# KyungMinJin/OTPose

Hardware: AMD Instinct MI355X
Metric: frames/sec at 384x288, 5-frame window, batch 16; heatmap max-abs delta vs ref (higher is better)
Workload: dtype f32 storage+accumulate / f16x3 split products; 1 GPU; BASELINE configs[1]: batch 16 x 5-frame x 384x288, HRNet-W48 + DCN warp + ConvVideoTransformer, fp32 forward (eval), seeded synthetic weights; clips_per_gpu=16, parallelism=dp1, outputs_finite=True

## Files before the change

include/otpose_hip.h:

```cpp
#ifndef OTPOSE_HIP_H
#define OTPOSE_HIP_H

#include <stddef.h>

#ifdef __cplusplus
extern "C" {
#endif

#define OTP_OK 0
#define OTP_ERR_BAD_ARG (-1)
#define OTP_ERR_UNSUPPORTED (-2)
#define OTP_ERR_LAUNCH (-3)
#define OTP_ERR_WORKSPACE (-4)

#define OTP_DTYPE_F32 0
#define OTP_DTYPE_F16 1
#define OTP_DTYPE_BF16 2
#define OTP_DTYPE_F64 3

#define OTP_ACT_NONE 0
#define OTP_ACT_RELU 1
#define OTP_ACT_GELU 2

int otp_version(void);
// ... 101 lines not shown
int otp_conv3x3_small_supported(const otp_conv_desc* desc);
size_t otp_conv3x3_small_weight_bytes(int Cout, int Cin);
int otp_conv3x3_small_pack(const void* weight, void* wpacked, int Cout, int Cin, void* stream);
int otp_conv3x3_small(const void* in, const void* in2, const void* wpacked, const void* scale, const void* shift, void* out,
                      const otp_conv_desc* desc, void* stream);

size_t otp_conv2d_x3_weight_bytes(int Cout, int Cin, int k, int stride);
int otp_conv2d_x3_pack_weight(const void* weight, const void* scale, void* wpacked, int Cout, int Cin, int k, int stride,
                              void* stream);
int otp_conv2d_x3_supported(const otp_conv_desc* desc);
int otp_conv2d_x3(const void* in, const void* wpacked, const void* shift, const void* res, void* out,
                  const otp_conv_desc* desc, void* stream);

#define OTP_S8_F32_C4 1
#define OTP_S8_F32_NCHW 2
size_t otp_s8_bytes(int N, int C, int H, int W);
int otp_s8_pack(const void* in_f32, void* out_s8, void* out_c4, int N, int C, int H, int W, int in_ctot, int in_coff, void* stream);
int otp_s8_upsample_add(const void* const* lows, const int* factors, int nlow, const void* res, void* out_nchw, void* out_s8,
                        void* out_c4, int N, int C, int Hh, int Wh, int relu, int res_ctot, int res_coff, int out_ctot,
                        int out_coff, void* stream);
int otp_s8_upsample_add_ex(const void* const* lows, const int* factors, int nlow, const void* res, int res_layout, void* out_nchw,
                           void* out_s8, void* out_c4, int N, int C, int Hh, int Wh, int relu, int res_ctot, int res_coff,
                           int out_ctot, int out_coff, void* stream);
int otp_s8_unpack(const void* in_s8, void* out_f32, int N, int C, int H, int W, void* stream);
int otp_c4_unpack(const void* in_c4, void* out_f32, int N, int C, int H, int W, void* stream);
int otp_conv3x3_s8_supported(const otp_conv_desc* desc);
size_t otp_conv3x3_s8_weight_bytes(int Cout, int Cin);
int otp_conv3x3_s8_pack_weight(const void* weight, const void* scale, void* wpacked, int Cout, int Cin, void* stream);
int otp_conv3x3_s8(const void* in_s8, const void* wpacked, const void* shift, const void* res_c4, void* out_f32,
                   int out_f32_layout, void* out_s8, const otp_conv_desc* desc, void* stream);
int otp_conv3x3_s2_s8_supported(const otp_conv_desc* desc, int nchw_out);
int otp_conv3x3_s2_s8(const void* in_s8, const void* wpacked, const void* shift, const void* res_nchw, void* out_nchw,
                      void* out_s8, const otp_conv_desc* desc, void* stream);

int otp_conv2d_pack_weight_dgrad(const void* weight, void* wpacked, int Cout, int Cin, int kh, int kw, void* stream);
int otp_dilate(const void* in, void* out, int planes, int Hi, int Wi, int s, int H, int W, void* stream);
size_t otp_conv2d_wgrad_workspace(int Cin, int Cout);
int otp_conv2d_wgrad(const void* x, const void* grad_out, void* grad_weight, int N, int Cin, int H, int W, int Cout,
                     int kh, int kw, int stride, int pad, int dil, int x_ctot, int x_coff, int dy_ctot, int dy_coff,
                     void* workspace, size_t workspace_bytes, void* stream);
size_t otp_bn_workspace(int N, int C, int HW);
int otp_bn_train_forward(const void* x, const void* gamma, const void* beta, const void* res, void* y, void* save_mean,
                         void* save_rstd, void* running_mean, void* running_var, void* workspace, size_t workspace_bytes,
                         int N, int C, int HW, float eps, float momentum, int relu, int x_ctot, int x_coff, int res_ctot,
                         int res_coff, int y_ctot, int y_coff, void* stream);
int otp_bn_train_backward(const void* grad_y, const void* x, const void* y_relu, const void* save_mean,
                          const void* save_rstd, const void* gamma, void* grad_x, void* grad_res, void* grad_gamma,
                          void* grad_beta, void* workspace, size_t workspace_bytes, int N, int C, int HW, int dy_ctot,
                          int dy_coff, int x_ctot, int x_coff, int y_ctot, int y_coff, void* stream);
int otp_channel_sum(const void* a, void* out, void* workspace, size_t workspace_bytes, int N, int C, int HW, int a_ctot,
                    int a_coff, void* stream);

int otp_dcn_fused_supported(int Cin, int J, int H, int W, int ND);
size_t otp_dcn_fused_weight_bytes(int ND, int J);
int otp_dcn_fused_pack(const void* const* w_off, const void* const* w_mask, const void* const* w_dcn, const void* const* bias,
                       void* packed, int ND, int J, void* stream);
size_t otp_dcn_fused_workspace(int B, int H, int W);
int otp_dcn_fused_forward(const void* trans, const void* x, const void* packed, void* out, void* workspace,
                          size_t workspace_bytes, int B, int Cin, int J, int H, int W, const int* dilations, int ND, float alpha,
                          void* stream);

int otp_glue_total(const void* rough, void* total, void* squeezed, void* inter, void* flow_in, const void* pe,
                   int B, int J, int HW, void* stream);
int otp_glue_stack(const void* rough, const void* margin, const void* squeezed, const void* inter,
                   const void* ctx, const void* pe1, const void* pe2, void* x1, void* x2, void* prev_b,
                   int B, int J, int HW, void* stream);
// ... 249 lines not shown
```

otpose_amd/csrc/convs2.hip:

```cpp
#include "x3.h"
#include <cstdlib>

namespace {

constexpr int MAXJ = 4;

struct S2Plan {
    int N, C, H, W, HW, Ho, Wo, HWo, Cout, total;
    int out_ctot, out_coff, res_ctot, res_coff, act;
    float pre, post;
    int NTW, nN, nTiles, nChunks, tpx, NPT;
    int VR, W1, NIW, NV, pl;
    uint32_t mHWo, mWo, mW1, mVR;
    unsigned* rflag;
};

template <int NTW, bool NCHW, int NPT>
__global__ __launch_bounds__(256, 2) void convs2_kernel(const unsigned char* __restrict__ xs, const otp_u32x4* __restrict__ wpk,
                                                         const float* __restrict__ shift, const float* res, float* outf,
                                                         otp_u32x4* outs, const S2Plan P) {
    constexpr int BM = 64 * NPT;
    constexpr int WCH = otp_s8_wch(NTW);
    constexpr int WBYTES = WCH * 1024;
    constexpr int NBLK = OTP_S8_KS * NPT;
    constexpr int NM = 3 * NTW;
    extern __shared__ __attribute__((aligned(16))) unsigned char smem[];
    const int PL = P.pl;
    unsigned char* win = smem;
    unsigned char* wl = smem + 4 * PL;
    const int tid = threadIdx.x, lane = tid & 63;
    const int wave = __builtin_amdgcn_readfirstlane(tid >> 6);
    const int i16 = lane & 15, kl = lane >> 4;
    const bool upper = kl >= 2;

    const int xcd = (int)blockIdx.x & 7, jb = (int)blockIdx.x >> 3;
    const int tl_ = jb / P.nN, cb = jb - tl_ * P.nN;
    const int tile = xcd * P.tpx + tl_;
    if (tile >= P.nTiles) return;
    const int P0 = tile * BM;
    const int n0 = P0 / P.HWo, p0 = P0 - n0 * P.HWo;
    const int y0 = (int)otp_magic_div((uint32_t)p0, P.mWo);
    const int Vf = n0 * P.VR + 2 * y0;
    const int imgB = P.C * P.HW * 4;
    const int co_blk = cb * NTW * 16;

    int voff[MAXJ];
    bool vlive[MAXJ];
#pragma unroll
    for (int j = 0; j < MAXJ; ++j) {
        const int v = 64 * (wave + 4 * j) + lane;
        vlive[j] = v < P.NV;
        const int r = (int)otp_magic_div((uint32_t)v, P.mW1), i = v - r * P.W1;
        const int V = Vf + r;
// ... 98 lines not shown
            const bool nb = blk + 2 < NBLK;
            const bool na = (NPT >= 2 ? p == NPT - 2 : true) && s + 1 < OTP_S8_KS;
            if (nb) load_b((blk + 2) % 3, blk + 2);
            if (na) load_a(sa ^ 1, s + 1);
#pragma unroll
            for (int t = 0; t < NTW; ++t) {
                acc[t][p] = OTP_X3_MFMA(al[sa][t], bh[cur], acc[t][p], 0, 0, 0);
                acc[t][p] = OTP_X3_MFMA(ah[sa][t], bl[cur], acc[t][p], 0, 0, 0);
                acc[t][p] = OTP_X3_MFMA(ah[sa][t], bh[cur], acc[t][p], 0, 0, 0);
            }
            if (!nb && !na) otp_s8_block_sched<NM, 0>();
            else if (nb && na) otp_s8_block_sched<NM, 2 + 2 * NTW>();
            else if (na) otp_s8_block_sched<NM, 2 * NTW>();
            else otp_s8_block_sched<NM, 2>();
            __builtin_amdgcn_sched_barrier(0);
        }
    };

    for (int c = 0; c < P.nChunks; ++c) {
        asm volatile("s_waitcnt vmcnt(0)" ::: "memory");
        __syncthreads();
        mfma_phase();
        if (c + 1 < P.nChunks) {
            __syncthreads();
            stage(c + 1);
        }
    }

    if (P.post != 1.f) {
#pragma unroll
        for (int t = 0; t < NTW; ++t)
#pragma unroll
            for (int p = 0; p < NPT; ++p) acc[t][p] = acc[t][p] * P.post;
    }
    if (!NCHW) {
        {
            bool bad = false;
#pragma unroll
            for (int t = 0; t < NTW; ++t)
#pragma unroll
                for (int p = 0; p < NPT; ++p)
#pragma unroll
                    for (int r = 0; r < 4; ++r) bad |= otp_out_of_range(acc[t][p][r]);
            otp_range_report(P.rflag, bad, OTP_RANGE_CONVS2);
        }
        if (P.act == OTP_ACT_RELU) {
#pragma unroll
            for (int t = 0; t < NTW; ++t)
#pragma unroll
                for (int p = 0; p < NPT; ++p)
#pragma unroll
                    for (int r = 0; r < 4; ++r) acc[t][p][r] = otp_relu(acc[t][p][r]);
        }
        otp_u32x4 rec[(NTW + 1) / 2][NPT][2];
#pragma unroll
        for (int t = 0; t < NTW; t += 2) {
            const bool paired = otp_tile_paired(co_blk, t, NTW, P.Cout);
            const int t1 = t + 1 < NTW ? t + 1 : t;
#pragma unroll
            for (int p = 0; p < NPT; ++p) {
                const float f[8] = {acc[t][p][0], acc[t][p][1], acc[t][p][2], acc[t][p][3],
                                    paired ? acc[t1][p][0] : 0.f, paired ? acc[t1][p][1] : 0.f,
                                    paired ? acc[t1][p][2] : 0.f, paired ? acc[t1][p][3] : 0.f};
                otp_x3_split8(f, rec[t >> 1][p][0], rec[t >> 1][p][1]);
            }
        }
// ... 108 lines not shown
        const int NV = window_records(P, bm);
        size_t lds = (size_t)4 * NV * 16 + otp_s8_wch(P.NTW) * 1024;
        if (nchw && lds < (size_t)P.NTW * 16 * (bm + 4) * 4) lds = (size_t)P.NTW * 16 * (bm + 4) * 4;
        if (NV <= 64 * 4 * MAXJ && lds <= 80 * 1024) {
            P.NV = NV;
            found = true;
            if ((long)P.nTiles * P.nN >= 2 * 256 || npt == 1) break;
        }
    }
    if (!found) return false;
    {
        const int bm = 64 * P.NPT;
        P.nTiles = (P.total + bm - 1) / bm;
        P.NV = window_records(P, bm);
        if (P.NV > 64 * 4 * MAXJ) return false;
    }
    P.tpx = (P.nTiles + 7) / 8;
    P.pl = P.NV * 16;
    P.NIW = (P.NV + 63) / 64;
    P.mHWo = otp_magic(P.HWo); P.mWo = otp_magic(Wo); P.mW1 = otp_magic(P.W1); P.mVR = otp_magic(P.VR);
    if ((long)(P.HWo + 256) * P.HWo >= (1l << 32) || (long)P.HWo * Wo >= (1l << 32)) return false;
    if ((long)(d.N + 2) * P.VR * P.VR >= (1l << 32) || (long)(64 * 4 * MAXJ) * P.W1 >= (1l << 32)) return false;
    {
        const long span = (long)(64 * P.NPT) / P.HWo + 2;
        if (span * d.Cin * P.HW * 4 >= (1l << 31)) return false;
    }
    if ((size_t)d.N * d.out_ctot * P.HWo * 4 >= (1ull << 31) || (size_t)d.N * (d.res_ctot > 0 ? d.res_ctot : 1) * P.HWo * 4 >= (1ull << 31))
        return false;
    if ((size_t)P.nN * P.nChunks * otp_s8_wch(P.NTW) * 1024 >= (1ull << 31)) return false;
    if (P.HWo < 16) return false;
    return true;
}

template <int NTW, bool NCHW, int NPT>
int convs2_launch(const void* xs, const void* wpk, const float* shift, const float* res, float* outf, void* outs, const S2Plan& P,
                  hipStream_t st) {
    auto kern = convs2_kernel<NTW, NCHW, NPT>;
    size_t need = (size_t)4 * P.pl + otp_s8_wch(NTW) * 1024;
    if (NCHW && need < (size_t)NTW * 16 * (64 * NPT + 4) * 4) need = (size_t)NTW * 16 * (64 * NPT + 4) * 4;
    OTP_ALLOW_BIG_LDS(kern, need);
    hipLaunchKernelGGL(kern, dim3(8 * P.tpx * P.nN), dim3(256), need, st, static_cast<const unsigned char*>(xs),
                       static_cast<const otp_u32x4*>(wpk), shift, res, outf, static_cast<otp_u32x4*>(outs), P);
    return otp_launch_status();
}

}

extern "C" int otp_conv3x3_s2_s8_supported(const otp_conv_desc* desc, int nchw_out) {
    if (!desc) return 0;
    S2Plan P{};
    return convs2_plan(*desc, P, nchw_out != 0) ? 1 : 0;
}

extern "C" int otp_conv3x3_s2_s8(const void* in_s8, const void* wpacked, const void* shift, const void* res_nchw, void* out_nchw,
                                 void* out_s8, const otp_conv_desc* desc, void* stream) {
    if (!in_s8 || !wpacked || !desc || (!out_nchw) == (!out_s8)) return OTP_ERR_BAD_ARG;
    if (res_nchw && !out_nchw) return OTP_ERR_BAD_ARG;
    const otp_conv_desc& d = *desc;
    if (d.N <= 0 || d.Cin <= 0 || d.Cout <= 0 || d.H <= 0 || d.W <= 0) return OTP_ERR_BAD_ARG;
    if (out_nchw && d.out_ctot < d.out_coff + d.Cout) return OTP_ERR_BAD_ARG;
    if (res_nchw && d.res_ctot < d.res_coff + d.Cout) return OTP_ERR_BAD_ARG;
    if ((reinterpret_cast<uintptr_t>(in_s8) | reinterpret_cast<uintptr_t>(wpacked) | reinterpret_cast<uintptr_t>(out_nchw) |
         reinterpret_cast<uintptr_t>(out_s8) | reinterpret_cast<uintptr_t>(res_nchw) | reinterpret_cast<uintptr_t>(shift)) & 15)
        return OTP_ERR_UNSUPPORTED;
    S2Plan P{};
    const bool nchw = out_nchw != nullptr;
    if (!convs2_plan(d, P, nchw)) return OTP_ERR_UNSUPPORTED;
    P.rflag = otp_range_word();
    auto st = static_cast<hipStream_t>(stream);
    auto fs = static_cast<const float*>(shift);
    auto fr = static_cast<const float*>(res_nchw);
    auto fo = static_cast<float*>(out_nchw);
#define OTP_C2_GO(NTW_, NCHW_, NPT_) return convs2_launch<NTW_, NCHW_, NPT_>(in_s8, wpacked, fs, fr, fo, out_s8, P, st)
#define OTP_C2_NPT(NPT_)                                                     \
    if (P.NPT == NPT_) {                                                     \
        if (P.NTW == 2) { if (nchw) OTP_C2_GO(2, true, NPT_); OTP_C2_GO(2, false, NPT_); } \
        if (nchw) OTP_C2_GO(3, true, NPT_);                                  \
        OTP_C2_GO(3, false, NPT_);                                           \
    }
    OTP_C2_NPT(4)
    OTP_C2_NPT(2)
    OTP_C2_NPT(1)
#undef OTP_C2_NPT
#undef OTP_C2_GO
    return OTP_ERR_UNSUPPORTED;
}
```

otpose_amd/engine.py:

```python
from __future__ import annotations

import ctypes
import dataclasses
import os
import sys
import warnings
from typing import Callable, List, Optional, Tuple

import torch

from . import hip, ops
from .ops import ACT_GELU, ACT_NONE, ACT_RELU, View

def _pair(v):
    return (int(v), int(v)) if isinstance(v, int) else (int(v[0]), int(v[1]))


def plain_conv(cv, k, stride=1, pad="same", dil=1, groups=1, bias=False, cin=None, cout=None) -> bool:
    if pad == "same":
        pad = (dil or 1) * (k // 2)
    return (cv.kernel_size == (k, k) and (stride is None or cv.stride == (stride, stride))
            and (pad is None or tuple(cv.padding) == (pad, pad)) and (dil is None or tuple(cv.dilation) == (dil, dil))
            and (groups is None or cv.groups == groups) and (bias is None or (cv.bias is not None) == bias)
            and (cin is None or cv.in_channels == cin) and (cout is None or cv.out_channels == cout))
# ... 61 lines not shown
    def __init__(self, s8=None, c4=None, nchw_needed=False):
        self.s8, self.c4, self.nchw_needed = s8, c4, nchw_needed


class InferenceEngine:
    h16 = False

    def __init__(self, model, batch: int, device, use_graph: bool | None = None, stream_set: int = 0, inp=None, margin=None):
        routes = Routes.from_env()
        self._init(device, routes, routes.use_graph if use_graph is None else use_graph, stream_set)
        self.B = batch
        self.model = model
        cfg = model.cfg
        self.J = model.num_joints
        self.F = getattr(model, "window_frames", 5)
        self.W_img, self.H_img = cfg.MODEL.IMAGE_SIZE
        self.h, self.w = model.pe_h, model.pe_w
        self._given = (inp, margin)
        self.param_version = self._param_version()
        with torch.no_grad():
            self._build()

    def _init(self, device, routes: Routes, use_graph: bool, stream_set: int = 0):
        device = torch.device(device)
        if device.type != "cuda" or not torch.cuda.is_available():
            raise RuntimeError("otpose_amd.OTPose runs on an MI355X through libotpose_hip.so; "
                               f"got device '{device}' (there is no CPU or PyTorch-op fallback)")
        self.lib, self.dev, self.routes = hip.lib(), device, routes
        self.model, self.B, self.inp, self.margin = None, 0, None, None
        self.ops: List[Callable] = []
        self._pair_s8 = {}
        self.l1_pairs = 0
        self._aux = {}
        self._keep = []
        self._bufs = []
        self._stream = None
        self.use_graph, self.graph = use_graph, None
        self._exact = False
        self._sid = 0
        self._side = hip.side_streams(device, 3, 4 * stream_set) if routes.multi_stream else []

    @classmethod
    def bare(cls, device, multi_stream=False):
        self = cls.__new__(cls)
        self._init(device, dataclasses.replace(Routes.from_env(), multi_stream=bool(multi_stream)), use_graph=False)
        return self

    use_x3 = property(lambda self: self.routes.use_x3)
    use_dcn_fused = property(lambda self: self.routes.use_dcn_fused)
    multi_stream = property(lambda self: self.routes.multi_stream)
    f32_tail = property(lambda self: self.routes.f32_tail)
    range_check = property(lambda self: self.routes.range_check)
    half_products = property(lambda self: self.h16 and self.routes.use_x3 and self.routes.h16_tail)

    @property
    def s8_here(self) -> bool:
        return self.routes.use_s8 and not self._exact

    @property
    def s2_here(self) -> bool:
        return self.routes.use_s8 and not self._exact and self.routes.s8_stride2

    def matches(self, x) -> bool:
        return (x.shape[0] == self.B and x.device == self.dev and tuple(x.shape[2:]) == (self.H_img, self.W_img)
                and self._param_version() == self.param_version)

# ... 32 lines not shown
        return cin >= 32 and cin % 8 == 0 and cout16 >= 48 and ((cout16 + 47) // 48) * 48 <= 1.15 * cout16

    def _emit(self, fn):
        self.ops.append((fn, self._sid))

    def fork(self, sids):
        if not self.multi_stream:
            return
        sids = [s for s in sids if 0 < s <= len(self._side)]

        def run():
            main = torch.cuda.current_stream(self.dev)
            for s_ in sids:
                self._side[s_ - 1].wait_stream(main)
        self.ops.append((run, -1))

    def join(self, sids):
        if not self.multi_stream:
            return
        sids = [s for s in sids if 0 < s <= len(self._side)]

        def run():
            main = torch.cuda.current_stream(self.dev)
            for s_ in sids:
                main.wait_stream(self._side[s_ - 1])
        self.ops.append((run, -1))

    def on_stream(self, sid):
        self._sid = sid if (self.multi_stream and 0 <= sid <= len(self._side)) else 0

    def call(self, fn, name, *args):
        def run():
            hip.check(fn(*args, self._stream), name)
        self._emit(run)

    def call_lazy_nchw(self, aux: Aux, fn, name, args_of, unpack=None):
        full, lean = args_of(True), args_of(False)
        if unpack is None:
            def run():
                hip.check(fn(*(full if aux.nchw_needed else lean), self._stream), name)
        else:
            s8_unpack = self.lib.otp_s8_unpack

            def run():
                hip.check(fn(*lean, self._stream), name)
                if aux.nchw_needed:
                    hip.check(s8_unpack(*unpack, self._stream), "otp_s8_unpack")
        self._emit(run)

    def _bn_fold(self, bn, bias=None):
        g, b = self.dev_param(bn.weight), self.dev_param(bn.bias)
        mu, var = self.dev_param(bn.running_mean), self.dev_param(bn.running_var)
        sc = (g / torch.sqrt(var + bn.eps)).contiguous()
        sh = b - mu * sc
        if bias is not None:
            sh = sh + self.dev_param(bias) * sc
        sh = sh.contiguous()
        self._keep += [sc, sh]
        return sc, sh

    def conv(self, inp: View, weight, out: View, stride=1, pad=0, dil=1, bn=None, bias=None, act=ACT_NONE,
             res: View = None, in2: View = None, res_up=1, frame_split=0, cin=None, scale=None, shift=None):
        for v_ in (inp, in2, res):
            self._needs_nchw(v_)
        r = self.routes
        w = self.dev_param(weight)
        if w.dim() == 3:
            w = w.unsqueeze(-1)
        cout, cin_w, kh, kw = w.shape
        if bn is not None:
# ... 75 lines not shown

    def fuse_s8(self, lows, factors, res: View, tgt: View):
        n_, c_, hh, wh = tgt.t.shape
        if not self.s8_here or tgt.coff != 0 or tgt.C != c_ or c_ % 16 or wh % 4 or (hh * wh) % 4:
            return False
        if not ops.s8_conv_supported(ops.s8_conv_desc(n_, c_, c_, hh, wh, ACT_RELU)):
            return False
        r = self.routes
        raux = self._aux.get(id(res.t)) if (r.lazy_nchw and res.coff == 0 and res.C == c_ and res.ctot == c_) else None
        res_img = raux.s8 if raux is not None else None
        if res_img is None:
            self._needs_nchw(res)
        s8 = self.new(n_ * c_ * hh * wh)
        c4 = None if r.s8_residual else self.new(n_ * c_ * hh * wh)
        aux = self._aux[id(tgt.t)] = Aux(s8, c4)
        lp = (ctypes.c_void_p * len(lows))(*[hip.ptr(v.t) for v in lows])
        fp = (ctypes.c_int * len(lows))(*factors)
        self._keep += [lp, fp]
        self.call_lazy_nchw(aux, self.lib.otp_s8_upsample_add_ex, "otp_s8_upsample_add", lambda nchw: (
            lp, fp, len(lows), hip.ptr(res_img if res_img is not None else res.t), int(res_img is not None),
            hip.ptr(tgt.t) if nchw else None, hip.ptr(s8), hip.ptr(c4), n_, c_, hh, wh, 1, res.ctot, res.coff, tgt.ctot, tgt.coff))
        return True

    def s8_image(self, v: View, want_c4=False):
        n, c, h, w = v.t.shape
        if not self.routes.use_s8 or v.coff != 0 or v.C != c or c % 16 or (h * w) % 4:
            return None
        aux = self._aux.get(id(v.t))
        if aux is not None and aux.s8 is not None and (not want_c4 or aux.c4 is not None):
            return aux
        self._needs_nchw(v)
        s8 = aux.s8 if aux is not None and aux.s8 is not None else self.new(n * c * h * w)
        c4 = self.new(n * c * h * w) if want_c4 else None
        self.call(self.lib.otp_s8_pack, "otp_s8_pack", hip.ptr(v.t), hip.ptr(s8), hip.ptr(c4), n, c, h, w, v.ctot, v.coff)
        if aux is None:
            aux = self._aux[id(v.t)] = Aux(nchw_needed=True)
        aux.s8 = s8
        if c4 is not None:
            aux.c4 = c4
        return aux

    def s2_chain_s8(self, layers, x: View, act_last, res: View = None, out: View = None):
        if not self.s2_here:
            return None
        n, c, h, w = x.t.shape
        if x.coff != 0 or x.C != c:
            return None
        hh, ww, cin = h, w, c
        descs = []
        for li, (cv, bn, relu) in enumerate(layers):
            last = li == len(layers) - 1
            if not plain_conv(cv, 3, stride=2, cin=cin) or hh % 2 or ww % 2:
                return None
            co = cv.out_channels
            if last:
                if out is None:
                    out = View(self.new(n, co, hh // 2, ww // 2))
                d = ops.s8_s2_conv_desc(n, cin, co, hh, ww, act_last, out, res)
            else:
                d = ops.s8_s2_conv_desc(n, cin, co, hh, ww, ACT_RELU if relu else ACT_NONE)
            if not ops.s8_s2_conv_supported(d, last):
                return None
            descs.append(d)
            hh, ww, cin = hh // 2, ww // 2, co
        aux = self.s8_image(x)
        if aux is None:
            return None
        self._needs_nchw(res)
        cur = aux.s8
        hh, ww = h, w
        for (cv, bn, relu), d in zip(layers, descs):
            wp, sh = self._pack_s8(cv, bn, d)
            if d is descs[-1]:
                args = ops.conv3x3_s2_s8_args(cur, wp, sh, d, res, out)
            else:
                nxt = self.new(n * cv.out_channels * (hh // 2) * (ww // 2))
                args = ops.conv3x3_s2_s8_args(cur, wp, sh, d, out_s8=nxt)
                cur = nxt
            self.call(self.lib.otp_conv3x3_s2_s8, "otp_conv3x3_s2_s8", *args)
            hh, ww = hh // 2, ww // 2
        return out

    def _pack_s8(self, conv, bn, desc):
        sc, sh = self._bn_fold(bn)
        w = self.dev_param(conv.weight)
        e = ops.x3_weight_exponent(w, sc)
        desc.out_scale = 2.0 ** -e
        wp = ops.pack_s8_weight(w, sc, e)
        self._keep += [wp, desc]
        return wp, sh

    def conv_s8(self, x8, conv, bn, d, **outputs):
        wp, sh = self._pack_s8(conv, bn, d)
        self.call(self.lib.otp_conv3x3_s8, "otp_conv3x3_s8", *ops.conv3x3_s8_args(x8, wp, sh, d, **outputs))

    def conv_s8_lazy(self, x8, conv, bn, d, out: View, o8, res=None):
        wp, sh = self._pack_s8(conv, bn, d)
        aux = Aux(o8, nchw_needed=o8 is None or not self.routes.lazy_nchw)
        if o8 is not None:
            self._aux[id(out.t)] = aux
        self.call_lazy_nchw(aux, self.lib.otp_conv3x3_s8, "otp_conv3x3_s8", lambda nchw: ops.conv3x3_s8_args(
            x8, wp, sh, d, res, out.t if nchw else None, ops.S8_F32_NCHW, o8))

    def branch_s8(self, blocks, x: View, want_s8=False):
        n, c, h, w = x.t.shape
        if not self.s8_here or x.coff != 0 or x.C != c:
            return None
        for blk in blocks:
            convs = (getattr(blk, "conv1", None), getattr(blk, "conv2", None))
            if (getattr(blk, "downsample", None) is not None or hasattr(blk, "conv3")
                    or any(cv is None or not plain_conv(cv, 3, cin=c, cout=c) for cv in convs)):
                return None
        if not ops.s8_conv_supported(ops.s8_conv_desc(n, c, c, h, w, ACT_RELU)):
# ... 124 lines not shown
            sc, sh = self._bn_fold(blk.bn3)
            out = self.pointx_pair(y, c3.weight, sc, sh, res, nxt)
            if out is not None:
                return out
        return self.conv_bn(y, blk.conv3, blk.bn3, ACT_RELU, res=res)

    def hr_module(self, mod, xs: List[View], fork_in=True, join_out=True) -> List[View]:
        n = mod.num_branches
        xs = list(xs)
        r = self.routes
        if fork_in:
            self.fork(range(1, n))
        for i in range(n):
            self.on_stream(i)
            y = self.branch_s8(list(mod.branches[i]), xs[i], want_s8=i < len(mod.fuse_layers) - 1 and self.s2_here)
            if y is not None:
                xs[i] = y
                continue
            for blk in mod.branches[i]:
                xs[i] = self.basic_block(blk, xs[i])
        self.on_stream(0)
        self.join(range(1, n))
        if n == 1:
            return xs
        outs = []
        if self.s2_here:
            for j in range(min(n, len(mod.fuse_layers) - 1)):
                self.s8_image(xs[j])
        self.fork(range(1, len(mod.fuse_layers)))
        for i in range(len(mod.fuse_layers)):
            self.on_stream(i)
            terms = [j for j in range(n) if j != i]
            y = None
            ups = [j for j in terms if j > i]
            hi_w = xs[i].t.shape[3]
            if r.fuse_upsample and len(ups) >= 2 and hi_w % 4 == 0:
                terms = [j for j in terms if j < i]
            else:
                ups = []
            for idx, j in enumerate(terms):
                last = idx == len(terms) - 1 and not ups
                act = ACT_RELU if last else ACT_NONE
                res = xs[i] if y is None else y
                fl = mod.fuse_layers[i][j]
                tgt = y if y is not None else View(self.new(*xs[i].t.shape))
                if j > i:
                    f = 2 ** (j - i)
                    if f >= 2 and ((xs[j].t.shape[3] * f) % 4 == 0 or r.up_any_width):
                        low = self.conv_bn(xs[j], fl[0], fl[1], ACT_NONE)
                        if act == ACT_RELU and low.coff == 0 and low.C == low.ctot and self.fuse_s8([low], [f], res, tgt):
                            y = tgt
                            continue
                        self._needs_nchw(res)
                        self.call(self.lib.otp_upsample_add, "otp_upsample_add", *ops.upsample_add_args(low, res, tgt, f, act == ACT_RELU))
                        y = tgt
                    else:
                        y = self.conv_bn(xs[j], fl[0], fl[1], act, res=res, out=tgt, res_up=f)
                else:
                    chain = [(fl[k][0], fl[k][1], k < len(fl) - 1) for k in range(len(fl))]
                    if self.s2_chain_s8(chain, xs[j], act, res=res, out=tgt) is not None:
                        y = tgt
                        continue
                    t = xs[j]
                    for k in range(len(fl) - 1):
                        t = self.conv_bn(t, fl[k][0], fl[k][1], ACT_RELU)
                    y = self.conv_bn(t, fl[-1][0], fl[-1][1], act, res=res, out=tgt)
            if ups:
                res = xs[i] if y is None else y
                tgt = y if y is not None else View(self.new(*xs[i].t.shape))
                lows = [self.conv_bn(xs[j], mod.fuse_layers[i][j][0], mod.fuse_layers[i][j][1], ACT_NONE) for j in ups]
                factors = [2 ** (j - i) for j in ups]
                if self.fuse_s8(lows, factors, res, tgt):
                    outs.append(tgt)
                    continue
                self._needs_nchw(res)
                args, arrays = ops.upsample_add_multi_args(lows, factors, res, tgt, relu=True)
                self._keep += arrays
                self.call(self.lib.otp_upsample_add_multi, "otp_upsample_add_multi", *args)
                y = tgt
            outs.append(y)
        self.on_stream(0)
        if join_out:
            self.join(range(1, len(mod.fuse_layers)))
        return outs

    def hr_stages(self, net, x, width_change, new_branch, module, before_fork=None):
        ys = [x]
        for s in (2, 3, 4):
            trans = getattr(net, f"transition{s - 1}")
            live = [i for i, tr in enumerate(trans) if tr is not None]
            if before_fork is not None:
                before_fork(s, ys)
            self.fork(range(1, len(live)))
            xs = []
            for i, tr in enumerate(trans):
                if tr is None:
                    xs.append(ys[i])
                    continue
                self.on_stream(live.index(i))
                if isinstance(tr[0], torch.nn.Conv2d):
                    xs.append(width_change(s, ys[i], tr))
                else:
                    xs.append(new_branch(s, ys[-1], tr))
            self.on_stream(0)
            self.join(range(1, len(live)))
            ys = xs
            mods = list(getattr(net, f"stage{s}"))
            cont = False
            for mi, mod in enumerate(mods):
                fork_in, nxt = not cont, (mods[mi + 1] if mi + 1 < len(mods) else None)
                cont = (self.routes.chain_modules and nxt is not None and len(mod.fuse_layers) == nxt.num_branches
                        and mod.num_branches > 1)
                ys = module(s, mi, len(mods), mod, ys, fork_in, not cont)
        return ys

    def hrnet(self, net, x_in: View) -> View:
        c1 = net.conv1
# ... 393 lines not shown
```

otpose_amd/hip.py:

```python
from __future__ import annotations

import ctypes
import os
import threading
from ctypes import c_float, c_int, c_size_t, c_void_p

_HERE = os.path.dirname(os.path.abspath(__file__))
LIB_PATH = os.environ.get("OTPOSE_HIP_LIB") or os.path.join(_HERE, "csrc", "libotpose_hip.so")
_lib = None
_tls = threading.local()

OTP_OK = 0
_ERRORS = {
    -1: "OTP_ERR_BAD_ARG (null pointer or non-positive dimension)",
    -2: "OTP_ERR_UNSUPPORTED (shape / dtype / stride combination not implemented)",
    -3: "OTP_ERR_LAUNCH (HIP launch error)",
    -4: "OTP_ERR_WORKSPACE (workspace too small)",
}


class ConvDesc(ctypes.Structure):
    _fields_ = [(n, c_int) for n in (
        "N", "Cin", "H", "W", "Cout", "kh", "kw", "stride", "pad", "dil",
        "in_ctot", "in_coff", "in2_ctot", "in2_coff", "out_ctot", "out_coff",
# ... 47 lines not shown
    "otp_mdcn_backward": (c_int, [c_void_p] * 10 + [c_void_p, c_size_t] + [c_int] * 12 + [c_int, c_void_p]),
    "otp_deform_psroi_pool_forward": (c_int, [c_void_p] * 5 + [c_int] * 7 + [c_float] + [c_int] * 5 + [c_float, c_int, c_void_p]),
    "otp_deform_psroi_pool_backward_workspace": (c_size_t, [c_int] * 13),
    "otp_deform_psroi_pool_backward": (c_int, [c_void_p] * 7 + [c_int] * 7 + [c_float] + [c_int] * 5 + [c_float]
                                       + [c_void_p, c_size_t, c_int, c_void_p]),
    "otp_conv2d_pack_weight": (c_int, [c_void_p, c_void_p, c_int, c_int, c_int, c_int, c_void_p]),
    "otp_conv2d": (c_int, [c_void_p] * 7 + [ctypes.POINTER(ConvDesc), c_void_p]),
    "otp_conv2d_wino_weight_bytes": (c_size_t, [c_int, c_int]),
    "otp_conv2d_wino_pack_weight": (c_int, [c_void_p, c_void_p, c_int, c_int, c_void_p]),
    "otp_conv2d_wino_supported": (c_int, [ctypes.POINTER(ConvDesc)]),
    "otp_conv2d_wino_last_plan": (c_int, [ctypes.POINTER(c_int)]),
    "otp_conv2d_wino": (c_int, [c_void_p] * 6 + [ctypes.POINTER(ConvDesc), c_void_p]),
    "otp_conv3x3_small_supported": (c_int, [ctypes.POINTER(ConvDesc)]),
    "otp_conv3x3_small_weight_bytes": (c_size_t, [c_int, c_int]),
    "otp_conv3x3_small_pack": (c_int, [c_void_p, c_void_p, c_int, c_int, c_void_p]),
    "otp_conv3x3_small": (c_int, [c_void_p] * 6 + [ctypes.POINTER(ConvDesc), c_void_p]),
    "otp_conv2d_x3_weight_bytes": (c_size_t, [c_int, c_int, c_int, c_int]),
    "otp_conv2d_x3_pack_weight": (c_int, [c_void_p, c_void_p, c_void_p, c_int, c_int, c_int, c_int, c_void_p]),
    "otp_conv2d_x3_supported": (c_int, [ctypes.POINTER(ConvDesc)]),
    "otp_conv2d_x3": (c_int, [c_void_p] * 5 + [ctypes.POINTER(ConvDesc), c_void_p]),
    "otp_s8_bytes": (c_size_t, [c_int] * 4),
    "otp_s8_pack": (c_int, [c_void_p] * 3 + [c_int] * 6 + [c_void_p]),
    "otp_s8_upsample_add": (c_int, [ctypes.POINTER(c_void_p), ctypes.POINTER(c_int), c_int] + [c_void_p] * 4 + [c_int] * 9 + [c_void_p]),
    "otp_s8_upsample_add_ex": (c_int, [ctypes.POINTER(c_void_p), ctypes.POINTER(c_int), c_int, c_void_p, c_int] + [c_void_p] * 3
                               + [c_int] * 9 + [c_void_p]),
    "otp_s8_unpack": (c_int, [c_void_p, c_void_p] + [c_int] * 4 + [c_void_p]),
    "otp_c4_unpack": (c_int, [c_void_p, c_void_p] + [c_int] * 4 + [c_void_p]),
    "otp_conv3x3_s8_supported": (c_int, [ctypes.POINTER(ConvDesc)]),
    "otp_conv3x3_s8_weight_bytes": (c_size_t, [c_int, c_int]),
    "otp_conv3x3_s8_pack_weight": (c_int, [c_void_p] * 3 + [c_int, c_int, c_void_p]),
    "otp_conv3x3_s8": (c_int, [c_void_p] * 5 + [c_int, c_void_p, ctypes.POINTER(ConvDesc), c_void_p]),
    "otp_conv3x3_s2_s8_supported": (c_int, [ctypes.POINTER(ConvDesc), c_int]),
    "otp_conv3x3_s2_s8": (c_int, [c_void_p] * 6 + [ctypes.POINTER(ConvDesc), c_void_p]),
    "otp_conv2d_set_tile": (c_int, [c_int] * 4),
    "otp_conv2d_last_plan": (c_int, [ctypes.POINTER(c_int)]),
    "otp_conv2d_plan": (c_int, [ctypes.POINTER(ConvDesc), ctypes.POINTER(c_int)]),
    "otp_conv2d_pack_weight_dgrad": (c_int, [c_void_p, c_void_p, c_int, c_int, c_int, c_int, c_void_p]),
    "otp_dilate": (c_int, [c_void_p, c_void_p] + [c_int] * 6 + [c_void_p]),
    "otp_grad_sumsq_scratch": (c_size_t, []),
    "otp_grad_sumsq": (c_int, [c_void_p, c_size_t, c_void_p, c_void_p]),
    "otp_adamw_step": (c_int, [c_void_p] * 4 + [c_size_t] + [c_float] * 5 + [c_int, c_void_p, c_float, c_void_p]),
    "otp_pck_accuracy": (c_int, [c_void_p] * 4 + [c_int] * 4 + [c_float, c_void_p]),
    "otp_frames_u8_to_clip": (c_int, [c_void_p] * 2 + [c_int] * 4 + [c_float] * 6 + [c_void_p]),
    "otp_crop_clips_u8": (c_int, [c_void_p] + [c_int] * 3 + [c_void_p] * 4 + [c_int] * 4 + [c_float] * 6 + [c_void_p]),
    "otp_crop_clips_blur_u8": (c_int, [c_void_p] + [c_int] * 3 + [c_void_p] * 4 + [c_int] * 4 + [c_float] * 6
                               + [c_void_p] * 3),
    "otp_crop_clips_pair_u8": (c_int, [c_void_p] + [c_int] * 3 + [c_void_p] * 3 + [c_int] * 4 + [c_float] * 6 + [c_void_p]),
    "otp_pose_targets": (c_int, [c_void_p] * 6 + [c_int] * 7 + [c_void_p]),
    "otp_conv2d_wgrad_workspace": (c_size_t, [c_int] * 2),
    "otp_conv2d_wgrad": (c_int, [c_void_p] * 3 + [c_int] * 14 + [c_void_p, c_size_t, c_void_p]),
    "otp_bn_workspace": (c_size_t, [c_int] * 3),
    "otp_bn_train_forward": (c_int, [c_void_p] * 9 + [c_void_p, c_size_t] + [c_int] * 3 + [c_float, c_float] +
                             [c_int] * 7 + [c_void_p]),
    "otp_bn_train_backward": (c_int, [c_void_p] * 10 + [c_void_p, c_size_t] + [c_int] * 9 + [c_void_p]),
    "otp_channel_sum": (c_int, [c_void_p, c_void_p, c_void_p, c_size_t] + [c_int] * 5 + [c_void_p]),
    "otp_glue_total": (c_int, [c_void_p] * 6 + [c_int] * 3 + [c_void_p]),
    "otp_glue_stack": (c_int, [c_void_p] * 10 + [c_int] * 3 + [c_void_p]),
    "otp_glue_total_n": (c_int, [c_void_p] * 6 + [c_int] * 4 + [c_void_p]),
    "otp_glue_stack_n": (c_int, [c_void_p] * 10 + [c_int] * 4 + [c_void_p]),
    "otp_ln_channel": (c_int, [c_void_p] * 5 + [c_int] * 3 + [c_float, c_void_p]),
    "otp_dwconv_ln3": (c_int, [c_void_p] * 13 + [c_int] * 4 + [c_float, c_void_p]),
    "otp_chan_attn_workspace": (c_size_t, [c_int] * 4),
    "otp_dense_cc_supported": (c_int, [c_int] * 2),
    "otp_dense_cc_weight_bytes": (c_size_t, [c_int]),
    "otp_dense_cc_pack": (c_int, [c_void_p] * 4 + [c_int, c_void_p]),
    "otp_dense_cc": (c_int, [ctypes.POINTER(c_void_p)] * 4 + [c_int] * 4 + [c_void_p]),
# ... 193 lines not shown
```

otpose_amd/ops.py:

```python
from __future__ import annotations

import ctypes
import math
import os

import torch
from torch.autograd import Function

from . import hip
from .augment import FLIP_PAIRS

_DTYPE_F32 = 0


def _require_gpu(*tensors):
    for t in tensors:
        if t is not None and not t.is_cuda:
            raise NotImplementedError("otpose_amd operators run on the GPU only (no CPU path)")


def _check_f32(*tensors):
    for t in tensors:
        if t is not None and t.dtype != torch.float32:
            raise RuntimeError(f"otpose_amd HIP operators are built for float32, got {t.dtype}")
# ... 512 lines not shown
    _require_gpu(c4)
    out = torch.empty(n, c, h, w, dtype=torch.float32, device=c4.device)
    hip.check(hip.lib().otp_c4_unpack(hip.ptr(c4), hip.ptr(out), n, c, h, w, hip.stream_of(c4)), "otp_c4_unpack")
    return out


def s8_conv_supported(desc) -> bool:
    return bool(hip.lib().otp_conv3x3_s8_supported(desc))


def s8_conv_desc(n, cin, cout, h, w, act=ACT_NONE, out: View = None, res: View = None, stride=1):
    d = hip.ConvDesc()
    d.N, d.Cin, d.H, d.W, d.Cout = n, cin, h, w, cout
    d.kh = d.kw = 3
    d.stride, d.pad, d.dil = stride, 1, 1
    d.in_ctot, d.in_coff, d.in2_ctot, d.in2_coff = cin, 0, 0, 0
    d.out_ctot, d.out_coff = (out.ctot, out.coff) if out is not None else (cout, 0)
    d.res_ctot, d.res_coff = (res.ctot, res.coff) if res is not None else (0, 0)
    d.res_up = 1
    d.act, d.Ho, d.Wo, d.frame_split = act, h // stride, w // stride, 0
    return d


def s8_s2_conv_desc(n, cin, cout, h, w, act=ACT_NONE, out: View = None, res: View = None):
    return s8_conv_desc(n, cin, cout, h, w, act, out, res, stride=2)


def s8_s2_conv_supported(desc, nchw_out=True):
    return bool(hip.lib().otp_conv3x3_s2_s8_supported(desc, int(nchw_out)))


def conv3x3_s2_s8_args(in_s8, wpacked, shift, desc, res: View = None, out: View = None, out_s8=None):
    return (hip.ptr(in_s8), hip.ptr(wpacked), hip.ptr(shift), _vp(res), _vp(out), hip.ptr(out_s8), desc)


def conv3x3_s2_s8(x_s8, shape, weight, scale=None, shift=None, act=ACT_NONE, res=None, out="nchw"):
    _require_gpu(x_s8, weight)
    n, cin, h, w = shape
    cout = weight.shape[0]
    e = x3_weight_exponent(weight, scale)
    wp = pack_s8_weight(weight, scale, e)
    sh = shift.detach().contiguous().float() if shift is not None else None
    L = hip.lib()
    if out == "s8":
        assert res is None
        d = s8_s2_conv_desc(n, cin, cout, h, w, act)
        d.out_scale = 2.0 ** -e
        o8 = s8_empty(n, cout, h // 2, w // 2, x_s8.device)
        _launch(L.otp_conv3x3_s2_s8, "otp_conv3x3_s2_s8", conv3x3_s2_s8_args(x_s8, wp, sh, d, out_s8=o8), x_s8)
        return o8
    o = torch.empty(n, cout, h // 2, w // 2, dtype=torch.float32, device=x_s8.device)
    rv = View(res.contiguous()) if res is not None else None
    d = s8_s2_conv_desc(n, cin, cout, h, w, act, View(o), rv)
    d.out_scale = 2.0 ** -e
    _launch(L.otp_conv3x3_s2_s8, "otp_conv3x3_s2_s8", conv3x3_s2_s8_args(x_s8, wp, sh, d, rv, View(o)), x_s8)
    return o


def pack_s8_weight(weight, scale=None, k=0):
    _require_gpu(weight)
    _check_f32(weight)
    w = weight.detach().contiguous()
    cout, cin, kh, kw = w.shape
    assert kh == kw == 3
    L = hip.lib()
    nbytes = L.otp_conv3x3_s8_weight_bytes(cout, cin)
# ... 1123 lines not shown
```

Measured before the change: 3217 frames/s.

## Fuse upsampled low-branch sums and residual into stride-2 s8 conv epilogue

Adds a row-form variant of the stride-2 int8-split conv kernel. Its epilogue adds the residual and the nearest-upsampled outputs of the lower-resolution 1x1 branches, applies ReLU, and writes the packed s8 output, plus the NCHW output only when it is needed. The HRNet fuse-layer builder uses this path for rows whose width is not a multiple of 4 and that have lower branches to upsample. This replaces the separate upsample-add and repack launches and their extra memory round trips. In exchange it adds another template instantiation and more complex epilogue indexing, plus some plan/context bookkeeping in the engine.

```diff
diff --git a/include/otpose_hip.h b/include/otpose_hip.h
--- a/include/otpose_hip.h
+++ b/include/otpose_hip.h
@@ -157,6 +157,10 @@
 int otp_conv3x3_s2_s8_supported(const otp_conv_desc* desc, int nchw_out);
 int otp_conv3x3_s2_s8(const void* in_s8, const void* wpacked, const void* shift, const void* res_nchw, void* out_nchw,
                       void* out_s8, const otp_conv_desc* desc, void* stream);
+int otp_conv3x3_s2_s8_row_supported(const otp_conv_desc* desc, const int* factors, int nlow);
+int otp_conv3x3_s2_s8_row(const void* in_s8, const void* wpacked, const void* shift, const void* res_nchw,
+                          const void* const* lows, const int* factors, int nlow, void* out_nchw, void* out_s8,
+                          const otp_conv_desc* desc, void* stream);
 
 int otp_conv2d_pack_weight_dgrad(const void* weight, void* wpacked, int Cout, int Cin, int kh, int kw, void* stream);
 int otp_dilate(const void* in, void* out, int planes, int Hi, int Wi, int s, int H, int W, void* stream);
diff --git a/otpose_amd/csrc/convs2.hip b/otpose_amd/csrc/convs2.hip
--- a/otpose_amd/csrc/convs2.hip
+++ b/otpose_amd/csrc/convs2.hip
@@ -15,10 +15,19 @@
     unsigned* rflag;
 };
 
-template <int NTW, bool NCHW, int NPT>
+struct S2Row {
+    const float* low[3];
+    int sh[3];
+    int n;
+};
+
+enum { C2_S8 = 0, C2_NCHW = 1, C2_ROW = 2 };
+
+template <int NTW, int FORM, int NPT>
 __global__ __launch_bounds__(256, 2) void convs2_kernel(const unsigned char* __restrict__ xs, const otp_u32x4* __restrict__ wpk,
                                                          const float* __restrict__ shift, const float* res, float* outf,
-                                                         otp_u32x4* outs, const S2Plan P) {
+                                                         otp_u32x4* outs, const S2Plan P, const S2Row R) {
+    constexpr bool NCHW = FORM == C2_NCHW;
     constexpr int BM = 64 * NPT;
     constexpr int WCH = otp_s8_wch(NTW);
     constexpr int WBYTES = WCH * 1024;
@@ -183,6 +192,78 @@
         for (int t = 0; t < NTW; ++t)
 #pragma unroll
             for (int p = 0; p < NPT; ++p) acc[t][p] = acc[t][p] * P.post;
+    }
+    if constexpr (FORM == C2_ROW) {
+#pragma clang fp contract(off)
+        const unsigned fbytes = (unsigned)((size_t)P.N * P.out_ctot * P.HWo * 4);
+        const otp_rsrc rof = make_rsrc32(outf, outf ? fbytes : 0u);
+        const otp_rsrc rres = make_rsrc32(res ? res : reinterpret_cast<const float*>(xs),
+                                          res ? (unsigned)((size_t)P.N * P.res_ctot * P.HWo * 4) : 0u);
+        otp_rsrc rl[3];
+        int hwl[3];
+#pragma unroll
+        for (int k = 0; k < 3; ++k) {
+            const bool on = k < R.n;
+            hwl[k] = on ? P.HWo >> (2 * R.sh[k]) : 0;
+            rl[k] = make_rsrc32(on ? R.low[k] : reinterpret_cast<const float*>(xs), (unsigned)((size_t)P.N * P.Cout * hwl[k] * 4));
+        }
+        const bool relu = P.act == OTP_ACT_RELU;
+        bool bad = false;
+#pragma unroll
+        for (int p = 0; p < NPT; ++p) {
+            int m = (wave * NPT + p) * 16 + i16;
+            const bool pv = P0 + m < P.total;
+            if (!pv) m = P.total - 1 - P0;
+            const int q = p0 + m;
+            const int dn = (int)otp_magic_div((uint32_t)q, P.mHWo), pi = q - dn * P.HWo;
+            const int y = (int)otp_magic_div((uint32_t)pi, P.mWo), x = pi - y * P.Wo;
+            const int n = n0 + dn;
+            const int rb = ((n * P.res_ctot + P.res_coff) * P.HWo + pi) * 4;
+            const int ob = ((n * P.out_ctot + P.out_coff) * P.HWo + pi) * 4;
+            int lb[3];
+#pragma unroll
+            for (int k = 0; k < 3; ++k)
+                lb[k] = k < R.n ? (n * P.Cout * hwl[k] + (y >> R.sh[k]) * (P.Wo >> R.sh[k]) + (x >> R.sh[k])) * 4 : 0;
+#pragma unroll
+            for (int t = 0; t < NTW; t += 2) {
+                const bool paired = otp_tile_paired(co_blk, t, NTW, P.Cout);
+                const bool tav = co_blk + 16 * t < P.Cout;
+                float f[8];
+#pragma unroll
+                for (int h = 0; h < 2; ++h) {
+                    const int tt = (h && t + 1 < NTW) ? t + 1 : t;
+                    const bool live = pv && (h ? paired : tav);
+#pragma unroll
+                    for (int r = 0; r < 4; ++r) {
+                        const int ch = ch0[tt] + r;
+                        float v = acc[tt][p][r];
+                        asm("" : "+v"(v));
+                        v = v + (res ? bload(rres, live ? rb + ch * P.HWo * 4 : OTP_OOB, 0) : 0.f);
+#pragma unroll
+                        for (int k = 0; k < 3; ++k)
+                            if (k < R.n) v = v + bload(rl[k], live ? lb[k] + ch * hwl[k] * 4 : OTP_OOB, 0);
+                        if (!h || paired) bad |= otp_out_of_range(v);
+                        if (relu) v = fmaxf(v, 0.f);
+                        if (outf) bstore(v, rof, live ? ob + ch * P.HWo * 4 : OTP_OOB, 0);
+                        f[4 * h + r] = (!h || paired) ? v : 0.f;
+                    }
+                }
+                otp_u32x4 hi, lo;
+                otp_x3_split8(f, hi, lo);
+                const int so = (ch0[t] >> 3) * 2 * P.HWo * 16;
+                if (paired) {
+                    const int o = offS[p] != OTP_OOB ? offS[p] + so : OTP_OOB;
+                    __builtin_amdgcn_raw_buffer_store_b128(hi, rs8, o, 0, 0);
+                    __builtin_amdgcn_raw_buffer_store_b128(lo, rs8, o, P.HWo * 16, 0);
+                } else {
+                    const int o = (tav && offS[p] != OTP_OOB) ? offS[p] + so + 8 * ((ch0[t] >> 2) & 1) : OTP_OOB;
+                    __builtin_amdgcn_raw_buffer_store_b64((otp_u32x2){hi[0], hi[1]}, rs8, o, 0, 0);
+                    __builtin_amdgcn_raw_buffer_store_b64((otp_u32x2){lo[0], lo[1]}, rs8, o, P.HWo * 16, 0);
+                }
+            }
+        }
+        otp_range_report(P.rflag, bad, OTP_RANGE_CONVS2);
+        return;
     }
     if (!NCHW) {
         {
@@ -357,15 +438,16 @@
     return true;
 }
 
-template <int NTW, bool NCHW, int NPT>
+template <int NTW, int FORM, int NPT>
 int convs2_launch(const void* xs, const void* wpk, const float* shift, const float* res, float* outf, void* outs, const S2Plan& P,
-                  hipStream_t st) {
-    auto kern = convs2_kernel<NTW, NCHW, NPT>;
+                  const S2Row& R, hipStream_t st) {
+    constexpr bool NCHW = FORM == C2_NCHW;
+    auto kern = convs2_kernel<NTW, FORM, NPT>;
     size_t need = (size_t)4 * P.pl + otp_s8_wch(NTW) * 1024;
     if (NCHW && need < (size_t)NTW * 16 * (64 * NPT + 4) * 4) need = (size_t)NTW * 16 * (64 * NPT + 4) * 4;
     OTP_ALLOW_BIG_LDS(kern, need);
     hipLaunchKernelGGL(kern, dim3(8 * P.tpx * P.nN), dim3(256), need, st, static_cast<const unsigned char*>(xs),
-                       static_cast<const otp_u32x4*>(wpk), shift, res, outf, static_cast<otp_u32x4*>(outs), P);
+                       static_cast<const otp_u32x4*>(wpk), shift, res, outf, static_cast<otp_u32x4*>(outs), P, R);
     return otp_launch_status();
 }
 
@@ -396,12 +478,13 @@
     auto fs = static_cast<const float*>(shift);
     auto fr = static_cast<const float*>(res_nchw);
     auto fo = static_cast<float*>(out_nchw);
-#define OTP_C2_GO(NTW_, NCHW_, NPT_) return convs2_launch<NTW_, NCHW_, NPT_>(in_s8, wpacked, fs, fr, fo, out_s8, P, st)
+    const S2Row R{};
+#define OTP_C2_GO(NTW_, FORM_, NPT_) return convs2_launch<NTW_, FORM_, NPT_>(in_s8, wpacked, fs, fr, fo, out_s8, P, R, st)
 #define OTP_C2_NPT(NPT_)                                                     \
     if (P.NPT == NPT_) {                                                     \
-        if (P.NTW == 2) { if (nchw) OTP_C2_GO(2, true, NPT_); OTP_C2_GO(2, false, NPT_); } \
-        if (nchw) OTP_C2_GO(3, true, NPT_);                                  \
-        OTP_C2_GO(3, false, NPT_);                                           \
+        if (P.NTW == 2) { if (nchw) OTP_C2_GO(2, C2_NCHW, NPT_); OTP_C2_GO(2, C2_S8, NPT_); } \
+        if (nchw) OTP_C2_GO(3, C2_NCHW, NPT_);                               \
+        OTP_C2_GO(3, C2_S8, NPT_);                                           \
     }
     OTP_C2_NPT(4)
     OTP_C2_NPT(2)
@@ -410,3 +493,63 @@
 #undef OTP_C2_GO
     return OTP_ERR_UNSUPPORTED;
 }
+
+namespace {
+bool convs2_row_terms(const S2Plan& P, const void* const* lows, const int* factors, int nlow, S2Row& R) {
+    if (nlow < 0 || nlow > 3 || (nlow > 0 && !factors)) return false;
+    R.n = nlow;
+    for (int k = 0; k < nlow; ++k) {
+        const int f = factors[k];
+        if ((f != 2 && f != 4 && f != 8) || P.Ho % f || P.Wo % f) return false;
+        R.sh[k] = f == 2 ? 1 : (f == 4 ? 2 : 3);
+        R.low[k] = lows ? static_cast<const float*>(lows[k]) : nullptr;
+    }
+    return true;
+}
+}
+
+extern "C" int otp_conv3x3_s2_s8_row_supported(const otp_conv_desc* desc, const int* factors, int nlow) {
+    if (!desc) return 0;
+    S2Plan P{};
+    S2Row R{};
+    return (convs2_plan(*desc, P, false) && convs2_row_terms(P, nullptr, factors, nlow, R)) ? 1 : 0;
+}
+
+extern "C" int otp_conv3x3_s2_s8_row(const void* in_s8, const void* wpacked, const void* shift, const void* res_nchw,
+                                     const void* const* lows, const int* factors, int nlow, void* out_nchw, void* out_s8,
+                                     const otp_conv_desc* desc, void* stream) {
+    if (!in_s8 || !wpacked || !desc || !out_s8 || nlow < 0 || nlow > 3 || (nlow > 0 && (!lows || !factors))) return OTP_ERR_BAD_ARG;
+    const otp_conv_desc& d = *desc;
+    if (d.N <= 0 || d.Cin <= 0 || d.Cout <= 0 || d.H <= 0 || d.W <= 0) return OTP_ERR_BAD_ARG;
+    if (out_nchw && d.out_ctot < d.out_coff + d.Cout) return OTP_ERR_BAD_ARG;
+    if (res_nchw && d.res_ctot < d.res_coff + d.Cout) return OTP_ERR_BAD_ARG;
+    uintptr_t lowbits = 0;
+    for (int k = 0; k < nlow; ++k) {
+        if (!lows[k]) return OTP_ERR_BAD_ARG;
+        lowbits |= reinterpret_cast<uintptr_t>(lows[k]);
+    }
+    if (((reinterpret_cast<uintptr_t>(in_s8) | reinterpret_cast<uintptr_t>(wpacked) | reinterpret_cast<uintptr_t>(out_nchw) |
+          reinterpret_cast<uintptr_t>(out_s8) | reinterpret_cast<uintptr_t>(res_nchw) | reinterpret_cast<uintptr_t>(shift)) & 15) ||
+        (lowbits & 3))
+        return OTP_ERR_UNSUPPORTED;
+    S2Plan P{};
+    S2Row R{};
+    if (!convs2_plan(d, P, false) || !convs2_row_terms(P, lows, factors, nlow, R)) return OTP_ERR_UNSUPPORTED;
+    if (!out_nchw) { P.out_ctot = d.Cout; P.out_coff = 0; }
+    if (!res_nchw) { P.res_ctot = 0; P.res_coff = 0; }
+    P.rflag = otp_range_word();
+    auto st = static_cast<hipStream_t>(stream);
+    auto fs = static_cast<const float*>(shift);
+    auto fr = static_cast<const float*>(res_nchw);
+    auto fo = static_cast<float*>(out_nchw);
+#define OTP_C2_NPT(NPT_)                                                                                     \
+    if (P.NPT == NPT_) {                                                                                     \
+        if (P.NTW == 2) return convs2_launch<2, C2_ROW, NPT_>(in_s8, wpacked, fs, fr, fo, out_s8, P, R, st); \
+        return convs2_launch<3, C2_ROW, NPT_>(in_s8, wpacked, fs, fr, fo, out_s8, P, R, st);                 \
+    }
+    OTP_C2_NPT(4)
+    OTP_C2_NPT(2)
+    OTP_C2_NPT(1)
+#undef OTP_C2_NPT
+    return OTP_ERR_UNSUPPORTED;
+}
diff --git a/otpose_amd/engine.py b/otpose_amd/engine.py
--- a/otpose_amd/engine.py
+++ b/otpose_amd/engine.py
@@ -117,6 +117,9 @@
         self._pair_s8 = {}
         self.l1_pairs = 0
         self._aux = {}
+        self.plan = []
+        self._ctx = ""
+        self._s2_out = set()
         self._keep = []
         self._bufs = []
         self._stream = None
@@ -215,10 +218,12 @@
     def call(self, fn, name, *args):
         def run():
             hip.check(fn(*args, self._stream), name)
+        self.plan.append((name, self._ctx))
         self._emit(run)
 
     def call_lazy_nchw(self, aux: Aux, fn, name, args_of, unpack=None):
         full, lean = args_of(True), args_of(False)
+        self.plan.append((name, self._ctx))
         if unpack is None:
             def run():
                 hip.check(fn(*(full if aux.nchw_needed else lean), self._stream), name)
@@ -360,7 +365,11 @@
         self._needs_nchw(v)
         s8 = aux.s8 if aux is not None and aux.s8 is not None else self.new(n * c * h * w)
         c4 = self.new(n * c * h * w) if want_c4 else None
+        ctx = self._ctx
+        if id(v.t) in self._s2_out:
+            self._ctx = "s2fed"
         self.call(self.lib.otp_s8_pack, "otp_s8_pack", hip.ptr(v.t), hip.ptr(s8), hip.ptr(c4), n, c, h, w, v.ctot, v.coff)
+        self._ctx = ctx
         if aux is None:
             aux = self._aux[id(v.t)] = Aux(nchw_needed=True)
         aux.s8 = s8
@@ -368,8 +377,12 @@
             aux.c4 = c4
         return aux
 
-    def s2_chain_s8(self, layers, x: View, act_last, res: View = None, out: View = None):
-        if not self.s2_here:
+    def _row_form(self) -> bool:
+        return self.s2_here and self.routes.fuse_upsample and self.routes.lazy_nchw
+
+    def s2_chain_s8(self, layers, x: View, act_last, res: View = None, out: View = None, row=False, lows=(), factors=(),
+                    dry=False):
+        if not self.s2_here or (row and not self._row_form()):
             return None
         n, c, h, w = x.t.shape
         if x.coff != 0 or x.C != c:
@@ -382,23 +395,39 @@
                 return None
             co = cv.out_channels
             if last:
-                if out is None:
+                if out is None and not dry:
                     out = View(self.new(n, co, hh // 2, ww // 2))
                 d = ops.s8_s2_conv_desc(n, cin, co, hh, ww, act_last, out, res)
             else:
                 d = ops.s8_s2_conv_desc(n, cin, co, hh, ww, ACT_RELU if relu else ACT_NONE)
-            if not ops.s8_s2_conv_supported(d, last):
+            if not (ops.s8_s2_row_supported(d, factors) if (row and last) else ops.s8_s2_conv_supported(d, last)):
+                return None
+            if row and last and ((out is not None and (out.coff != 0 or out.C != co)) or any(v.coff or v.C != v.ctot for v in lows)):
                 return None
             descs.append(d)
             hh, ww, cin = hh // 2, ww // 2, co
+        if dry:
+            return True if (self.routes.use_s8 and c % 16 == 0 and (h * w) % 4 == 0) else None
         aux = self.s8_image(x)
         if aux is None:
             return None
         self._needs_nchw(res)
+        if self._ctx.startswith("row") and not self._ctx.endswith("+s2"):
+            self._ctx += "+s2"
         cur = aux.s8
         hh, ww = h, w
         for (cv, bn, relu), d in zip(layers, descs):
             wp, sh = self._pack_s8(cv, bn, d)
+            if d is descs[-1] and row:
+                for v in lows:
+                    self._needs_nchw(v)
+                o8 = self.new(n * cv.out_channels * (hh // 2) * (ww // 2))
+                oaux = self._aux[id(out.t)] = Aux(o8)
+                both = [ops.conv3x3_s2_s8_row_args(cur, wp, sh, d, o8, res, lows, factors, out if nchw else None)
+                        for nchw in (False, True)]
+                self._keep += [arr for _, arrays in both for arr in arrays]
+                self.call_lazy_nchw(oaux, self.lib.otp_conv3x3_s2_s8_row, "otp_conv3x3_s2_s8_row", lambda nchw: both[int(nchw)][0])
+                break
             if d is descs[-1]:
                 args = ops.conv3x3_s2_s8_args(cur, wp, sh, d, res, out)
             else:
@@ -407,6 +436,7 @@
                 cur = nxt
             self.call(self.lib.otp_conv3x3_s2_s8, "otp_conv3x3_s2_s8", *args)
             hh, ww = hh // 2, ww // 2
+        self._s2_out.add(id(out.t))
         return out
 
     def _pack_s8(self, conv, bn, desc):
@@ -597,6 +627,9 @@
             self.on_stream(i)
             terms = [j for j in range(n) if j != i]
             y = None
+            self._ctx = f"row{i}"
+            if i >= 1 and self.fuse_row_s8(mod, xs, i, outs):
+                continue
             ups = [j for j in terms if j > i]
             hi_w = xs[i].t.shape[3]
             if r.fuse_upsample and len(ups) >= 2 and hi_w % 4 == 0:
@@ -644,10 +677,45 @@
                 self.call(self.lib.otp_upsample_add_multi, "otp_upsample_add_multi", *args)
                 y = tgt
             outs.append(y)
+        self._ctx = ""
         self.on_stream(0)
         if join_out:
             self.join(range(1, len(mod.fuse_layers)))
         return outs
+
+    def fuse_row_s8(self, mod, xs, i, outs) -> bool:
+        n = mod.num_branches
+        ups = list(range(i + 1, n))
+        factors = [2 ** (j - i) for j in ups]
+        if not self._row_form() or len(ups) > 3:
+            return False
+        if not ups or xs[i].t.shape[3] % 4 == 0:
+            return False
+        fls = mod.fuse_layers[i]
+        chain_of = lambda j: [(fls[j][k][0], fls[j][k][1], k < len(fls[j]) - 1) for k in range(len(fls[j]))]
+        nb, cb, hb, wb = xs[i].t.shape
+        for j in ups:
+            cv, hl, wl = fls[j][0], xs[j].t.shape[2], xs[j].t.shape[3]
+            if not plain_conv(cv, 1, cout=cb) or hl * 2 ** (j - i) != hb or wl * 2 ** (j - i) != wb:
+                return False
+        if self.s2_chain_s8(chain_of(i - 1), xs[i - 1], ACT_RELU, res=xs[i], row=True, factors=factors, dry=True) is None:
+            return False
+        tgt = View(self.new(*xs[i].t.shape))
+        y = None
+        for j in range(i - 1):
+            res = xs[i] if y is None else y
+            if self.s2_chain_s8(chain_of(j), xs[j], ACT_NONE, res=res, out=tgt) is None:
+                t = xs[j]
+                for k in range(len(fls[j]) - 1):
+                    t = self.conv_bn(t, fls[j][k][0], fls[j][k][1], ACT_RELU)
+                self.conv_bn(t, fls[j][-1][0], fls[j][-1][1], ACT_NONE, res=res, out=tgt)
+            y = tgt
+        lows = [self.conv_bn(xs[j], fls[j][0], fls[j][1], ACT_NONE) for j in ups]
+        done = self.s2_chain_s8(chain_of(i - 1), xs[i - 1], ACT_RELU, res=xs[i] if y is None else y, out=tgt, row=True, lows=lows,
+                                factors=factors)
+        assert done is not None
+        outs.append(tgt)
+        return True
 
     def hr_stages(self, net, x, width_change, new_branch, module, before_fork=None):
         ys = [x]
diff --git a/otpose_amd/hip.py b/otpose_amd/hip.py
--- a/otpose_amd/hip.py
+++ b/otpose_amd/hip.py
@@ -103,6 +103,9 @@
     "otp_conv3x3_s8": (c_int, [c_void_p] * 5 + [c_int, c_void_p, ctypes.POINTER(ConvDesc), c_void_p]),
     "otp_conv3x3_s2_s8_supported": (c_int, [ctypes.POINTER(ConvDesc), c_int]),
     "otp_conv3x3_s2_s8": (c_int, [c_void_p] * 6 + [ctypes.POINTER(ConvDesc), c_void_p]),
+    "otp_conv3x3_s2_s8_row_supported": (c_int, [ctypes.POINTER(ConvDesc), ctypes.POINTER(c_int), c_int]),
+    "otp_conv3x3_s2_s8_row": (c_int, [c_void_p] * 4 + [ctypes.POINTER(c_void_p), ctypes.POINTER(c_int), c_int, c_void_p, c_void_p,
+                                      ctypes.POINTER(ConvDesc), c_void_p]),
     "otp_conv2d_set_tile": (c_int, [c_int] * 4),
     "otp_conv2d_last_plan": (c_int, [ctypes.POINTER(c_int)]),
     "otp_conv2d_plan": (c_int, [ctypes.POINTER(ConvDesc), ctypes.POINTER(c_int)]),
diff --git a/otpose_amd/ops.py b/otpose_amd/ops.py
--- a/otpose_amd/ops.py
+++ b/otpose_amd/ops.py
@@ -568,6 +568,36 @@
 
 def conv3x3_s2_s8_args(in_s8, wpacked, shift, desc, res: View = None, out: View = None, out_s8=None):
     return (hip.ptr(in_s8), hip.ptr(wpacked), hip.ptr(shift), _vp(res), _vp(out), hip.ptr(out_s8), desc)
+
+
+def s8_s2_row_supported(desc, factors=()):
+    fp = (ctypes.c_int * max(len(factors), 1))(*[int(f) for f in factors])
+    return bool(hip.lib().otp_conv3x3_s2_s8_row_supported(desc, fp, len(factors)))
+
+
+def conv3x3_s2_s8_row_args(in_s8, wpacked, shift, desc, out_s8, res: View = None, lows=(), factors=(), out: View = None):
+    lp = (ctypes.c_void_p * max(len(lows), 1))(*[_vp(v) for v in lows])
+    fp = (ctypes.c_int * max(len(lows), 1))(*[int(f) for f in factors])
+    return (hip.ptr(in_s8), hip.ptr(wpacked), hip.ptr(shift), _vp(res), lp, fp, len(lows), _vp(out), hip.ptr(out_s8), desc), (lp, fp)
+
+
+def conv3x3_s2_s8_row(x_s8, shape, weight, scale=None, shift=None, act=ACT_NONE, res=None, lows=(), want_nchw=False):
+    _require_gpu(x_s8, weight)
+    n, cin, h, w = shape
+    cout = weight.shape[0]
+    e = x3_weight_exponent(weight, scale)
+    wp = pack_s8_weight(weight, scale, e)
+    sh = shift.detach().contiguous().float() if shift is not None else None
+    o = torch.empty(n, cout, h // 2, w // 2, dtype=torch.float32, device=x_s8.device) if want_nchw else None
+    o8 = s8_empty(n, cout, h // 2, w // 2, x_s8.device)
+    rv = View(res.contiguous()) if res is not None else None
+    lows = [t.contiguous() for t in lows]
+    d = s8_s2_conv_desc(n, cin, cout, h, w, act, View(o) if want_nchw else None, rv)
+    d.out_scale = 2.0 ** -e
+    args, _keep = conv3x3_s2_s8_row_args(x_s8, wp, sh, d, o8, rv, [View(t) for t in lows], [(h // 2) // t.shape[2] for t in lows],
+                                         View(o) if want_nchw else None)
+    _launch(hip.lib().otp_conv3x3_s2_s8_row, "otp_conv3x3_s2_s8_row", args, x_s8)
+    return o8, o
 
 
 def conv3x3_s2_s8(x_s8, shape, weight, scale=None, shift=None, act=ACT_NONE, res=None, out="nchw"):
```

Result: no change. 3199 frames/s (-0.6%).
